# AlexanderDzhoganov/sphereflake-raytracer

Hardware: AMD Instinct MI355X
Metric: Mrays/sec into G-buffer at 1920x1080 depth-8; frame time ms (higher is better)
Workload: dtype f32

## Files before the change

### sphereflake-raytracer_amd/csrc/sf_capi.hip

```cpp
#include <hip/hip_runtime.h>

#include <cfloat>
#include <cmath>
#include <cstdlib>
#include <cstring>
#include <new>
#include <utility>
#include <vector>

#include "sf_build_id.h"
#include "sf_internal.h"
#include "sphereflake/sf.h"

extern "C" __global__ void sf_trace_wave1(FrameArgs a, uint32_t* overflow_list, uint32_t* overflow_count);
extern "C" __global__ void sf_trace_wave2(FrameArgs a, uint32_t* overflow_list, uint32_t* overflow_count);
extern "C" __global__ void sf_trace_wave4(FrameArgs a, uint32_t* overflow_list, uint32_t* overflow_count);
extern "C" __global__ void sf_trace_queue1(FrameArgs a);
extern "C" __global__ void sf_trace_queue1c(FrameArgs a);
extern "C" __global__ void sf_trace_queue1t(FrameArgs a);
extern "C" __global__ void sf_trace_frames1(FrameBatch b);
extern "C" __global__ void sf_trace_queue1g(FrameArgs a);
extern "C" __global__ void sf_trace_queue1s(FrameArgs a);
extern "C" __global__ void sf_trace_queue2(FrameArgs a);
extern "C" __global__ void sf_trace_queue4(FrameArgs a);
// ... 827 lines not shown
    a.min_t = min_t;
    a.hit_index = hidx;
    a.tile_trace = c->tile_trace;
    a.counters = c->ovf_counters;
    a.overflow_list = c->ovf_list;
    a.parity = c->parity;
    if (c->tile_trace) {
        const size_t ntr = (size_t)((c->W + 7) / 8) * ((c->H + 7) / 8);
        a.phase_sums = c->tile_trace + 3 * ntr;
    }

    uint32_t ntiles = a.tiles_x * tile_rows;
    const uint32_t blocks = (ntiles + SF_WAVES_PER_BLOCK - 1) / SF_WAVES_PER_BLOCK;
    if (p.kernel == SF_KERNEL_PER_RAY) {
        a.max_depth = 31;
        hipLaunchKernelGGL(sf_trace_ray, dim3(blocks), dim3(256), 0, s, a);
        SF_HIP(c, hipGetLastError());
    } else {
        const bool autod = p.max_depth == 0;
        bool bounded = false;
        uint32_t levels = frame_levels(c, &bounded);
        if (!autod) bounded = bounded && p.max_depth >= levels;
        a.max_depth = autod ? levels : p.max_depth;
        const size_t lds = (size_t)SF_LDS_WAVE_FLOATS(a.max_depth) * 4;
        uint32_t* cnt = c->ovf_counters + c->parity;
        const uint32_t wpb = c->waves_per_block;
        const dim3 block(64 * wpb);
        const bool front_first = (c->flags & (SF_FLAG_NO_OCCL_CULL | SF_FLAG_NO_FRONT_FIRST)) == 0u;
        const bool tie_inline = bounded && c->persistent && front_first && c->tie_inline;
        if (tie_inline) a.flags |= SF_FLAG_TIE_INLINE;
        if (c->persistent) {
            const uint32_t lean_off = SF_FLAG_DIAG_HALF | SF_FLAG_DIAG_HALF_SEL | SF_FLAG_DIAG_UNITS |
                                      SF_FLAG_DIAG_FORCE_RETRACE | SF_FLAG_PRIO_FLAT;
            const bool plain = c->lean && wpb == 1 && band_count == 1u && !a.compact && !a.packed && !a.emit_aux &&
                               !a.tile_trace;
            const bool lean_ok = plain && (a.flags & lean_off) == 0u;
            const void* kern = wpb == 1 ? (const void*)sf_trace_queue1g
                             : wpb == 2 ? (c->compact ? (const void*)sf_trace_queue2c : (const void*)sf_trace_queue2)
                                        : (const void*)sf_trace_queue4;
            const int key = (int)(wpb * 64 + a.max_depth) | (c->compact ? 1 << 20 : 0);
            if (c->occ_key != key) {
                int nb = 0;
                SF_HIP(c, hipOccupancyMaxActiveBlocksPerMultiprocessor(&nb, kern, (int)block.x, wpb * lds));
                c->occ_blocks = nb < 1 ? 1 : nb;
                c->occ_blocks_lean = c->occ_blocks;
                c->occ_blocks_pair = c->occ_blocks;
                if (wpb == 1) {
                    SF_HIP(c, hipOccupancyMaxActiveBlocksPerMultiprocessor(&nb, (const void*)sf_trace_queue1t, (int)block.x, lds));
                    c->occ_blocks_lean = nb < 1 ? 1 : nb;
                    SF_HIP(c, hipOccupancyMaxActiveBlocksPerMultiprocessor(&nb, (const void*)sf_trace_queue1, (int)block.x, lds));
                    c->occ_blocks_pair = nb < 1 ? 1 : nb;
                    SF_HIP(c, hipOccupancyMaxActiveBlocksPerMultiprocessor(&nb, (const void*)sf_trace_queue1c, (int)block.x, lds));
                    if (nb >= 1 && nb < c->occ_blocks_pair) c->occ_blocks_pair = nb;
                }
                c->occ_key = key;
            }
            const uint32_t pair_off = lean_off & ~SF_FLAG_DIAG_FORCE_RETRACE;
            const uint32_t pair_grid = (uint32_t)(c->occ_blocks_pair > c->occ_blocks_lean ? c->occ_blocks_pair
// ... 1810 lines not shown
```

### sphereflake-raytracer_amd/csrc/sf_internal.h

```cpp
#pragma once

#include <stdint.h>

#if defined(__HIPCC__) || defined(__HIP__)
#define SF_HD __host__ __device__
#else
#define SF_HD
#endif

#define SF_DEPTH_TABLE 33
#ifndef SF_OCCL_MARGIN
#define SF_OCCL_MARGIN 0x1.8p-9f
#endif
#define SF_TILE 8
#define SF_WAVES_PER_BLOCK 4
#ifndef SF_WAVES_PER_EU
#define SF_WAVES_PER_EU 8
#endif
#ifndef SF_PAIR_WAVES_PER_EU
#define SF_PAIR_WAVES_PER_EU 7
#endif
#ifndef SF_TRACE_WAVES
#define SF_TRACE_WAVES 1
#endif
#define SF_LDS_ROOT 16
#define SF_LDS_CONE 8
#define SF_LDS_PLANE 38
#define SF_LDS_COLS 27
#define SF_LDS_TABLE (SF_LDS_PLANE + 3 * SF_LDS_COLS)
#define SF_LDS_E 32
#define SF_LDS_LEVEL (SF_LDS_TABLE + SF_LDS_E + 1)
#define SF_LDS_WAVE_FLOATS(levels) (SF_LDS_ROOT + SF_LDS_CONE + ((levels) - 1) * SF_LDS_LEVEL)
#define SF_RAYS_CSTACK (3 * 64)
#define SF_LDS_RAYS_FLOATS(levels) (SF_LDS_WAVE_FLOATS((levels) + 1) + (levels) * SF_RAYS_CSTACK)

#define SF_QUEUES 32u
// ... 226 lines not shown
```

### sphereflake-raytracer_amd/csrc/sf_kernels.hip

```cpp
#include <hip/hip_runtime.h>
#include <float.h>
#include <stddef.h>
#include <stdint.h>

#include "sf_internal.h"

#pragma clang fp contract(off)

#define SF_MAX_LEVELS 31

namespace {

__device__ __forceinline__ uint64_t wave_ballot(bool p) { return __builtin_amdgcn_ballot_w64(p); }

__device__ __forceinline__ float rsqrtps_x86(float x, const uint32_t* __restrict__ lut)
{
    const uint32_t b = __float_as_uint(x);
    const uint32_t E = (b >> 23) & 0xffu;
    const uint32_t key = ((E & 1u) << 10) | ((b & 0x7fffffu) >> 13);
    const int32_t E0 = (E & 1u) ? 127 : 128;
    const int32_t k = ((int32_t)E - E0) / 2;
    uint32_t r = (uint32_t)((int32_t)lut[key] - k * (1 << 23));
    if ((b & 0x7fffffffu) > 0x7f800000u) r = b | 0x00400000u;
    else if (E == 0u) r = (b & 0x80000000u) | 0x7f800000u;
// ... 501 lines not shown
    const float tlx = sel_mask(t_lo, -__builtin_inff(), tinym);
    const float th = hb ? thx : __builtin_inff();
    const float tl = hb ? tlx : __builtin_inff();
    uint64_t exm = wave_ballot(th < T);
    const uint64_t undm = wave_ballot(sel_mask(tl, __builtin_inff(), exm) < T);
    if (undm) {
        const float te = near_root_exact(tca, d2, R2b);
        exm |= undm & wave_ballot(te < T);
    }
    return exm;
}

__device__ __forceinline__ bool child_expands(float cx, float cy, float cz, float cc, float dx, float dy, float dz,
                                              float actv, float R2b, float T, float Tfar)
{
    const float tca = (cx * dx + cy * dy) + cz * dz;
    const float d2 = cc - tca * tca;
    const float xs = R2b - d2;
    const bool hb = __builtin_fminf(__builtin_fminf(tca, xs), actv) >= 0.0f;
    const uint64_t hbm = wave_ballot(hb);
    return hbm != 0ull && lod_expands(tca, d2, xs, hb, hbm, R2b, T, Tfar) != 0ull;
}

template <bool ANYHIT, bool INDEX_ORDER = false>
__device__ __forceinline__ uint64_t accept_hits(HitState& h, uint64_t& ancm, uint32_t& status, bool flag_ties,
                                                const float4 pc, float tca, float d2, uint32_t dd, uint64_t hsm,
                                                uint32_t idx, float R2s)
{
    {
        const float xs = R2s - d2;
        float ts;
        if ((wave_ballot(!(xs >= 0x1p-96f)) & hsm) != 0ull) ts = near_root_exact(tca, d2, R2s);
        else ts = near_root_big(tca, xs);
        uint64_t accm = hsm & wave_ballot(ts < h.minT);
        if constexpr (ANYHIT) {
            uint32_t hd = (uint32_t)h.depth;
            sel_in_place(hd, dd, accm);
            h.depth = (int32_t)hd;
            return accm;
        }
        const uint64_t tie = hsm & wave_ballot(ts == h.minT);
        if constexpr (INDEX_ORDER) accm |= tie & ancm;
        else if (tie != 0ull) {
            accm |= tie & ancm;
            if (flag_ties && (tie & ~ancm) != 0ull) status |= SF_STATUS_TIE;
        }
        sel_in_place(h.minT, ts, accm);
        sel_in_place(h.cx, pc.x, accm);
        sel_in_place(h.cy, pc.y, accm);
        sel_in_place(h.cz, pc.z, accm);
        sel_in_place(h.index, idx, accm);
        uint32_t hd = (uint32_t)h.depth;
        sel_in_place(hd, dd, accm);
        h.depth = (int32_t)hd;
        ancm |= accm;
        return accm;
    }
}
template <bool ANYHIT, bool INDEX_ORDER = false>
__device__ __forceinline__ uint64_t accept_self(HitState& h, uint64_t& ancm, uint32_t& status, bool flag_ties,
                                                const float4 pc, float tca, float d2, uint32_t dd, float actv,
                                                uint32_t idx, float R2s)
{
    const uint64_t hsm = wave_ballot(__builtin_fminf(__builtin_fminf(tca, R2s - d2), actv) >= 0.0f);
    if (hsm) return accept_hits<ANYHIT, INDEX_ORDER>(h, ancm, status, flag_ties, pc, tca, d2, dd, hsm, idx, R2s);
    return 0ull;
}

template <bool ANYHIT>
__device__ __forceinline__ uint64_t occluded(float tca, float minT, float cull_t, float cull_r)
{
    float v = tca - minT;
    if constexpr (!ANYHIT) v = __builtin_fminf(v, tca - cull_t);
    return wave_ballot(v - SF_OCCL_MARGIN * tca > cull_r);
}

__device__ __forceinline__ void leaf_children(HitState& h, uint64_t& ancm, uint32_t& status, bool flag_ties,
                                              bool occl_cull, const float* tb, uint32_t Cl, float dx, float dy, float dz,
                                              float avx, uint32_t idx0, uint32_t dd, const float4 dc, const float4 dk,
                                              float cull_t)
{
    const float R2b = dc.x, R2s = dc.y, T = dc.w, Tfar = dk.z, cull_r = dk.y;
    while (Cl) {
        const uint32_t p = __builtin_ctz(Cl);
        __asm__("s_bitset0_b32 %0, %1" : "+s"(Cl) : "s"(p));
        const uint32_t c = p & 15u;
        lds_fence();
        const float4 pc = *reinterpret_cast<const float4*>(tb + c * 4u);
        const float tca = (pc.x * dx + pc.y * dy) + pc.z * dz;
        const float d2 = pc.w - tca * tca;
        const bool hs = __builtin_fminf(__builtin_fminf(tca, R2s - d2), avx) >= 0.0f;
        const uint64_t hsm = wave_ballot(hs);
        if (hsm == 0ull) continue;
        uint64_t amx = lod_expands(tca, d2, R2b - d2, hs, hsm, R2b, T, Tfar);
        if (amx == 0ull) continue;
        if (occl_cull) {
            amx &= ~occluded<false>(tca, h.minT, cull_t, cull_r);
            if (amx == 0ull) continue;
        }
        ancm &= ~accept_hits<false>(h, ancm, status, flag_ties, pc, tca, d2, dd, amx, idx0 + c, R2s);
    }
}

template <class Ray>
__device__ __forceinline__ void leaf_children_pair(Ray& ra, Ray& rb, uint64_t& ancA, uint64_t& ancB, uint32_t& status,
                                                   bool flag_ties, bool occl_cull, const float* tb, uint32_t Cl,
                                                   float avxA, float avxB, uint32_t idx0, uint32_t dd, const float4 dc,
                                                   const float4 dk, float cull_t)
{
    const float R2b = dc.x, R2s = dc.y, T = dc.w, Tfar = dk.z, cull_r = dk.y;
    while (Cl) {
        const uint32_t p = __builtin_ctz(Cl);
        __asm__("s_bitset0_b32 %0, %1" : "+s"(Cl) : "s"(p));
        const uint32_t c = p & 15u;
        lds_fence();
        const float4 pc = *reinterpret_cast<const float4*>(tb + c * 4u);
        const float tcaA = (pc.x * ra.dx + pc.y * ra.dy) + pc.z * ra.dz;
        const float tcaB = (pc.x * rb.dx + pc.y * rb.dy) + pc.z * rb.dz;
        const float d2A = pc.w - tcaA * tcaA;
        const float d2B = pc.w - tcaB * tcaB;
        const bool hsA = __builtin_fminf(__builtin_fminf(tcaA, R2s - d2A), avxA) >= 0.0f;
        const bool hsB = __builtin_fminf(__builtin_fminf(tcaB, R2s - d2B), avxB) >= 0.0f;
        const uint64_t hsmA = wave_ballot(hsA), hsmB = wave_ballot(hsB);
        if ((hsmA | hsmB) == 0ull) continue;
        uint64_t amxA = hsmA ? lod_expands(tcaA, d2A, R2b - d2A, hsA, hsmA, R2b, T, Tfar) : 0ull;
        uint64_t amxB = hsmB ? lod_expands(tcaB, d2B, R2b - d2B, hsB, hsmB, R2b, T, Tfar) : 0ull;
        if ((amxA | amxB) == 0ull) continue;
        if (occl_cull) {
            amxA &= ~occluded<false>(tcaA, ra.h.minT, cull_t, cull_r);
            amxB &= ~occluded<false>(tcaB, rb.h.minT, cull_t, cull_r);
        }
        if (amxA) ancA &= ~accept_hits<false>(ra.h, ancA, status, flag_ties, pc, tcaA, d2A, dd, amxA, idx0 + c, R2s);
        if (amxB) ancB &= ~accept_hits<false>(rb.h, ancB, status, flag_ties, pc, tcaB, d2B, dd, amxB, idx0 + c, R2s);
    }
}

struct LeafLevel {
    float4 dc;
    bool on;
};
struct ChildBuild {
    float x, y, z, w;
    uint32_t M, front;
    float4 dtc;
    bool leaf_level;
};
template <bool KP_CONE = false>
__device__ __forceinline__ ChildBuild build_children(const DeviceConsts* K, const TraverseLds& L, const BuildLane& B,
                                                     const float4 pc, const float* col, uint32_t cs, uint32_t ko,
                                                     float kp, uint32_t index_order)
{
    lds_fence();
    const float3 p0 = *reinterpret_cast<const float3*>(col);
    const float3 p1 = *reinterpret_cast<const float3*>(col + cs);
    const float3 p2 = *reinterpret_cast<const float3*>(col + 2u * cs);
    const float4 cn = *reinterpret_cast<const float4*>(L.cone());
// ... 244 lines not shown
    __device__ __forceinline__ int32_t depth(uint32_t flags) const
    {
        int32_t seed = -1;
        if ((flags & (SF_FLAG_NO_OCCL_CULL | SF_FLAG_NO_DEPTH_SEED)) == 0u) {
            const int32_t w = __builtin_amdgcn_readfirstlane(word);
            const int32_t o = __builtin_amdgcn_readfirstlane(own);
            const int32_t m = o > w ? o : w;
            seed = (m > 0 ? m : 0) & 31;
        }
        return __builtin_amdgcn_readfirstlane(seed);
    }
};
__device__ __forceinline__ int32_t stats_word(const FrameArgs& a)
{
    return __hip_atomic_load(&a.stats[0], __ATOMIC_RELAXED, __HIP_MEMORY_SCOPE_AGENT);
}

__device__ __forceinline__ uint32_t split_mask(uint32_t q, uint32_t idxB)
{
    const uint32_t m9 = (0x111u << ((q - idxB) & 3u)) & 0x1ffu;
    return m9 | (m9 << 16);
}

template <bool COMPACT = false, bool SPLIT = false, bool SHADOW = false, bool LEAFNODES = !(COMPACT || SPLIT || SHADOW)>
__device__ __forceinline__ void traverse_ray(const DeviceConsts* __restrict__ K, const float* root, float* __restrict__ Lbase,
                                             const float4 bcol, uint32_t levels, float dx, float dy, float dz, bool valid,
                                             HitState& h, int32_t& maxd, uint32_t& status, uint32_t K_flags,
                                             uint64_t* phase_sums = nullptr, uint32_t axl = 36u,
                                             uint64_t* tile_counts = nullptr, uint32_t split_q = 0u,
                                             uint32_t split_depth = 0u, int32_t seed = -1, float bound = FLT_MAX)
{
    const uint32_t lane = threadIdx.x & 63u;
    const TraverseLds L{ Lbase };
    const bool cone_cull = (K_flags & SF_FLAG_NO_CONE_CULL) == 0u;
    const bool occl_cull = (K_flags & SF_FLAG_NO_OCCL_CULL) == 0u;
    const bool front_first = (K_flags & (SF_FLAG_NO_OCCL_CULL | SF_FLAG_NO_FRONT_FIRST)) == 0u;
    SF_STAMP_DECL;

    reset_hit(h, SHADOW ? bound : FLT_MAX);
    uint64_t ancm = 0ull;

    const float rcx = root[9], rcy = root[10], rcz = root[11];
    const float rcc = (rcx * rcx + rcy * rcy) + rcz * rcz;
    uint64_t ex0m;
    {
        const float4 dt0 = depth_consts(K, 0u);
        const float tca = (rcx * dx + rcy * dy) + rcz * dz;
        const float d2 = rcc - tca * tca;
        const bool hb = valid && tca >= 0.0f && d2 <= dt0.x;
        const uint64_t hbm = wave_ballot(hb);
        if (hbm == 0ull) return;
        ex0m = lod_expands(tca, d2, dt0.x - d2, hb, hbm, dt0.x, dt0.w, depth_word_at(K, 0u, 6u));
        if (ex0m == 0ull) return;
    }
    maxd = 0;

    {
        const float ax = readlane_f(dx, axl), ay = readlane_f(dy, axl), az = readlane_f(dz, axl);
        stage_cone(L, lane, cone_cull, ax, ay, az, [&] { return cone_s2m(dx, dy, dz, ax, ay, az); });
    }

    float cull_t = depth_consts(K, (uint32_t)(seed > 0 ? seed : 0) + 1u).w;

    const BuildLane B = build_lane(bcol, lane, build_child(lane));

    uint32_t d = 0;
    uint32_t idxB = 1;

    auto self_test = [&](const float4 pc, float tca, float d2, uint32_t dd, float actv, uint32_t idx,
                         float R2s) -> uint64_t {
        return accept_self<SHADOW>(h, ancm, status, front_first, pc, tca, d2, dd, actv, idx, R2s);
    };

    const uint32_t lv32 = __builtin_amdgcn_readfirstlane(levels << 5);
    const uint32_t index_order = front_first ? 0u : 0x1ffu;
    auto expand = [&](const float4 pc, const float* col, uint32_t cs, uint32_t d, float actv,
                      float* tb, uint32_t ko, float kp, LeafLevel& lf) -> uint32_t {
        d = __builtin_amdgcn_readfirstlane(d);
        SF_COUNT(0, 1);
        SF_COUNT(7, __builtin_popcountll(wave_ballot(actv >= 0.0f)));
        const ChildBuild cb = build_children(K, L, B, pc, col, cs, ko, kp, index_order);
        lf.dc = cb.dtc;
        lf.on = false;
        if (ko < lv32) {
            *reinterpret_cast<float3*>(tb + B.slot) = make_float3(cb.x, cb.y, cb.z);
            *(B.bc == 3u ? tb + B.slot + 3u : L.cone() + 5u) = cb.w;
            lf.on = cb.leaf_level;
            return (cb.M & cb.front) | ((cb.M & ~cb.front) << 16);
        }
        {
            const float R2b = cb.dtc.x, T = cb.dtc.w, Tfar = depth_word_at(K, ko, 6u);
            uint32_t M = cb.M;
            while (M) {
                const uint32_t i = __builtin_ctz(M);
// ... 83 lines not shown
            if (occl_cull) {
                amx = exm & ~occluded<SHADOW>(tca, h.minT, cull_t, cull_r);
                SF_COUNT(13, 1);
                SF_COUNT(12, amx == 0ull ? 1 : 0);
                if (amx == 0ull) continue;
            }
            float avx = sel_mask(-1.0f, __builtin_inff(), amx);
            const uint64_t acc = self_test(pc, tca, d2, d + 1u, avx, idxB + c, dc.y);
            SF_STAMP(4);
            if constexpr (SHADOW) {
                if (acc != 0ull) {
                    amx &= ~acc;
                    avx = sel_mask(avx, -1.0f, acc);
                    actv = sel_mask(actv, -1.0f, acc);
                    sel_in_place(actbits, 0u, acc);
                    if (wave_ballot(actbits != 0u) == 0ull) break;
                    if (amx == 0ull) continue;
                }
            }
            if (wave_ballot(pc.w > dk.x) != 0ull) {
                SF_COUNT(4, 1);
                SF_COUNT(8, 1);
                SF_COUNT(9, __builtin_popcountll(amx));
                ancm &= wave_ballot(h.depth != (int32_t)d + 1);
                continue;
            }
            const float* const col = tcur + SF_LDS_PLANE + 3u * c;
            auto push = [&]() {
                stk_pc = writelane_s(C, d, stk_pc);
                stk_ix = writelane_s(idxB, d, stk_ix);
                {
                    const uint32_t bit = 2u << d;
                    uint32_t ab = actbits & ~bit;
                    sel_in_place(ab, ab | bit, amx);
                    actbits = ab;
                }
                idxB = 9u * (idxB + c) + 1u;
                d += 1u;
                actv = avx;
                tcur += SF_LDS_LEVEL;
                kofs += 1u << 5;
            };
            LeafLevel lf;
            if constexpr (LEAFNODES) {
                SF_STAMP(1);
                const uint32_t Cn = expand(pc, col, SF_LDS_COLS, d + 1u, avx, tcur + SF_LDS_LEVEL, kofs + (1u << 5),
                                           readlane_f(tca, axl), lf);
                if (lf.on && (Cn == 0u || (int32_t)d + 2 <= (maxd > seed ? maxd : seed))) {
                    SF_COUNT(10, 1);
                    SF_COUNT(11, __builtin_popcount(Cn));
                    leaf_children(h, ancm, status, front_first, occl_cull, tcur + SF_LDS_LEVEL, Cn, dx, dy, dz, avx,
                                  9u * (idxB + c) + 1u, d + 2u, lf.dc, depth_consts_at(K, kofs + (1u << 5) + 16u), cull_t);
                    ancm &= wave_ballot(h.depth != (int32_t)d + 1);
                    SF_STAMP(6);
                    continue;
                }
                push();
                C = Cn;
            } else {
                push();
                SF_STAMP(1);
                C = expand(pc, col, SF_LDS_COLS, d, avx, tcur, kofs, readlane_f(tca, axl), lf);
            }
            if constexpr (SPLIT) {
                if (d + 1u == split_depth) C &= split_mask(split_q, idxB);
            }
            if constexpr (LEAFNODES) R2c = lf.dc.x;
            else R2c = depth_consts_at(K, kofs).x;
            if (COMPACT && C != 0u) {
                __builtin_amdgcn_sched_barrier(0);
                const uint64_t actm = wave_ballot(avx > 0.0f);
                const uint32_t na = (uint32_t)__builtin_popcountll(actm);
                const uint32_t M = (C | (C >> 16)) & 0x1ffu;
                if (na <= 7u && __builtin_popcount(M) >= 3) {
                    const float R2b = depth_consts(K, d + 1u).x;
                    const uint32_t rank = __builtin_amdgcn_mbcnt_hi((uint32_t)(actm >> 32),
// ... 4 lines not shown
                    uint32_t ln = lane;
                    __asm__ volatile("" : "+v"(ln));
                    const uint32_t g = (ln * 37u) >> 8;
                    const uint32_t sl = ln - 7u * g;
                    const float4 q = *reinterpret_cast<const float4*>(sc + 4u * sl);
                    const bool ok = sl < na && g < 9u && ((M >> g) & 1u) != 0u;
                    const uint32_t gi = g < 9u ? g : 8u;
                    const float4 cg = *reinterpret_cast<const float4*>(L.table(d) + gi * 4u);
                    const float tca = (cg.x * q.x + cg.y * q.y) + cg.z * q.z;
                    const float d2 = cg.w - tca * tca;
                    const float xs = R2b - d2;
                    const uint64_t bal =
                        wave_ballot(__builtin_fminf(__builtin_fminf(tca, xs), ok ? __builtin_inff() : -1.0f) >= 0.0f);
                    const uint32_t kk = ln < 9u ? ln : 0u;
                    const uint64_t grp = (bal >> (7u * kk)) & 0x7full;
                    const uint32_t hitm = (uint32_t)wave_ballot(ln < 9u && grp != 0ull) & 0x1ffu;
                    const uint32_t keep = __builtin_amdgcn_readfirstlane(hitm);
                    C &= keep | (keep << 16);
                }
            }
            SF_STAMP(6);
            continue;
        }
        ancm &= wave_ballot(h.depth != (int32_t)d);
        if (d == 0u) break;
        d -= 1u;
        tcur -= SF_LDS_LEVEL;
        kofs -= 1u << 5;
        R2c = depth_consts_at(K, kofs).x;
        {
            const uint32_t pw = __builtin_amdgcn_readlane(stk_pc, d);
            C = pw;
            idxB = (uint32_t)__builtin_amdgcn_readlane(stk_ix, d);
        }
        actv = ((actbits >> d) & 1u) ? __builtin_inff() : -1.0f;
        SF_STAMP(5);
    }
    h.hit = h.depth >= 0;
    SF_STAMP_FLUSH(phase_sums);
#ifdef SF_COUNTS
    if (tile_counts) {
        auto sat = [](uint64_t v) { return v > 0xffffull ? 0xffffull : v; };
        *tile_counts = sat(ph_sum[0]) | (sat(ph_sum[1]) << 16) | (sat(ph_sum[1] - ph_sum[2]) << 32) | (sat(ph_sum[8]) << 48);
    }
#else
    (void)tile_counts;
#endif
}

struct PairRay {
    float dx, dy, dz;
    HitState h;
    float actv;
    uint32_t actbits;
};

__device__ __forceinline__ void traverse_pair(const DeviceConsts* __restrict__ K, const float* root, float* __restrict__ Lbase,
                                              const float4 bcol, uint32_t levels, PairRay& ra, PairRay& rb, bool validA,
                                              bool validB, int32_t& maxd, uint32_t& status, uint32_t K_flags,
                                              int32_t seed)
{
    const uint32_t lane = threadIdx.x & 63u;
    const uint32_t axl = 39u;
    const TraverseLds L{ Lbase };
    const bool cone_cull = (K_flags & SF_FLAG_NO_CONE_CULL) == 0u;
    const bool occl_cull = (K_flags & SF_FLAG_NO_OCCL_CULL) == 0u;
    const bool front_first = (K_flags & (SF_FLAG_NO_OCCL_CULL | SF_FLAG_NO_FRONT_FIRST)) == 0u;

    reset_hit(ra.h, FLT_MAX);
    reset_hit(rb.h, FLT_MAX);
    uint64_t ancA = 0ull, ancB = 0ull;

    const float rcx = root[9], rcy = root[10], rcz = root[11];
    const float rcc = (rcx * rcx + rcy * rcy) + rcz * rcz;
    uint64_t ex0A = 0ull, ex0B = 0ull;
    {
        const float4 dt0 = depth_consts(K, 0u);
        const float Tfar0 = depth_word_at(K, 0u, 6u);
        auto root_lod = [&](const PairRay& r, bool valid) -> uint64_t {
            const float tca = (rcx * r.dx + rcy * r.dy) + rcz * r.dz;
            const float d2 = rcc - tca * tca;
            const bool hb = valid && tca >= 0.0f && d2 <= dt0.x;
            const uint64_t hbm = wave_ballot(hb);
            if (hbm == 0ull) return 0ull;
            return lod_expands(tca, d2, dt0.x - d2, hb, hbm, dt0.x, dt0.w, Tfar0);
        };
        ex0A = root_lod(ra, validA);
        ex0B = root_lod(rb, validB);
        if ((ex0A | ex0B) == 0ull) return;
    }
    maxd = 0;

    const float ax = readlane_f(ra.dx, axl), ay = readlane_f(ra.dy, axl), az = readlane_f(ra.dz, axl);
    {
        auto s2m_of = [&](const PairRay& r) -> float {
            const float cx_ = r.dy * az - r.dz * ay, cy_ = r.dz * ax - r.dx * az, cz_ = r.dx * ay - r.dy * ax;
            const float s2 = (cx_ * cx_ + cy_ * cy_) + cz_ * cz_;
            const bool fwd = (r.dx * ax + r.dy * ay) + r.dz * az > 0.0f;
            return fwd ? s2 : 1.0f;
        };
        uint32_t ln = lane;
        __asm__ volatile("" : "+v"(ln));
        stage_cone(L, ln, cone_cull, ax, ay, az, [&] { return __builtin_fmaxf(s2m_of(ra), s2m_of(rb)); });
    }

    float cull_t = depth_consts(K, (uint32_t)(seed > 0 ? seed : 0) + 1u).w;

    const BuildLane B = build_lane(bcol, lane, build_child(lane));

    uint32_t d = 0;
    uint32_t idxB = 1;

    auto self_test = [&](PairRay& r, uint64_t& ancm, const float4 pc, float tca, float d2, uint32_t dd, float actv,
                         uint32_t idx, float R2s) {
        accept_self<false>(r.h, ancm, status, front_first, pc, tca, d2, dd, actv, idx, R2s);
    };

    const uint32_t lv32 = __builtin_amdgcn_readfirstlane(levels << 5);
    const uint32_t index_order = front_first ? 0u : 0x1ffu;
    auto expand = [&](const float4 pc, const float* col, uint32_t cs, float* tb, uint32_t ko, float kp, auto kp_cone,
                      float actvA, float actvB, LeafLevel& lf) -> uint32_t {
        const ChildBuild cb = build_children<decltype(kp_cone)::value>(K, L, B, pc, col, cs, ko, kp, index_order);
        lf.dc = cb.dtc;
        lf.on = false;
        if (ko < lv32) {
            *reinterpret_cast<float3*>(tb + B.slot) = make_float3(cb.x, cb.y, cb.z);
            *(B.bc == 3u ? tb + B.slot + 3u : L.cone() + 5u) = cb.w;
            lf.on = cb.leaf_level;
            return (cb.M & cb.front) | ((cb.M & ~cb.front) << 16);
        }
        {
            const float R2b = cb.dtc.x, T = cb.dtc.w, Tfar = depth_word_at(K, ko, 6u);
            uint32_t M = cb.M;
            while (M) {
                const uint32_t i = __builtin_ctz(M);
                M &= ~(1u << i);
                const float cx = readlane_f(cb.x, 32u + i), cy = readlane_f(cb.y, 32u + i);
                const float cz = readlane_f(cb.z, 32u + i), cc = readlane_f(cb.w, 32u + i);
                auto passes = [&](const PairRay& r, float actv) -> bool {
                    return child_expands(cx, cy, cz, cc, r.dx, r.dy, r.dz, actv, R2b, T, Tfar);
                };
                if (passes(ra, actvA) || passes(rb, actvB)) {
                    status |= SF_STATUS_OVERFLOW;
                    break;
                }
            }
            return 0u;
        }
    };

    uint32_t stk_pc = 0u, stk_ix = 0u;
    float* tcur = L.table(0u);
    uint32_t kofs = 1u << 5;
    float R2c = depth_consts_at(K, kofs).x;
    uint32_t C = 0u;

    auto dfs_one = [&](const uint32_t base) {
        for (;;) {
            d = __builtin_amdgcn_readfirstlane(d);
            if (C) {
                const uint32_t p = __builtin_ctz(C);
                __asm__("s_bitset0_b32 %0, %1" : "+s"(C) : "s"(p));
                const uint32_t c = p & 15u;
                const float4 dc = depth_consts_at(K, kofs);
                lds_fence();
                const float4 pc = *reinterpret_cast<const float4*>(tcur + c * 4u);
                const float tca = (pc.x * ra.dx + pc.y * ra.dy) + pc.z * ra.dz;
                const float d2 = pc.w - tca * tca;
                const float xs = R2c - d2;
                const bool hb = __builtin_fminf(__builtin_fminf(tca, xs), ra.actv) >= 0.0f;
                const uint64_t hbm = wave_ballot(hb);
                if (hbm == 0ull) continue;
                const float4 dk = depth_consts_at(K, kofs + 16u);
                const float Tfar = dk.z;
                const float cull_r = dk.y;
                const uint64_t exm = lod_expands(tca, d2, xs, hb, hbm, dc.x, dc.w, Tfar);
                if (exm == 0ull) continue;
                if ((int32_t)d + 1 > maxd) {
                    maxd = (int32_t)d + 1;
                    if ((int32_t)d + 1 > seed) cull_t = depth_consts_at(K, kofs + (1u << 5)).w;
                }
                uint64_t amx = exm;
                if (occl_cull) {
                    amx = exm & ~occluded<false>(tca, ra.h.minT, cull_t, cull_r);
                    if (amx == 0ull) continue;
                }
                const float avx = sel_mask(-1.0f, __builtin_inff(), amx);
                self_test(ra, ancA, pc, tca, d2, d + 1u, avx, idxB + c, dc.y);
                if (wave_ballot(pc.w > dk.x) != 0ull) {
                    ancA &= wave_ballot(ra.h.depth != (int32_t)d + 1);
                    continue;
                }
                LeafLevel lf;
                const uint32_t Cn = expand(pc, tcur + SF_LDS_PLANE + 3u * c, SF_LDS_COLS, tcur + SF_LDS_LEVEL,
                                           kofs + (1u << 5), 0.0f, BoolC<true>(), avx, rb.actv, lf);
                if (lf.on && (Cn == 0u || (int32_t)d + 2 <= (maxd > seed ? maxd : seed))) {
                    leaf_children(ra.h, ancA, status, front_first, occl_cull, tcur + SF_LDS_LEVEL, Cn, ra.dx, ra.dy, ra.dz,
                                  avx, 9u * (idxB + c) + 1u, d + 2u, lf.dc, depth_consts_at(K, kofs + (1u << 5) + 16u), cull_t);
                    ancA &= wave_ballot(ra.h.depth != (int32_t)d + 1);
                    continue;
                }
                stk_pc = writelane_s(C, d, stk_pc);
                stk_ix = writelane_s(idxB, d, stk_ix);
                {
                    const uint32_t bit = 2u << d;
                    uint32_t ab = ra.actbits & ~bit;
                    sel_in_place(ab, ab | bit, amx);
                    ra.actbits = ab;
                }
                idxB = 9u * (idxB + c) + 1u;
                d += 1u;
                ra.actv = avx;
                tcur += SF_LDS_LEVEL;
                kofs += 1u << 5;
                C = Cn;
                R2c = lf.dc.x;
                continue;
            }
            ancA &= wave_ballot(ra.h.depth != (int32_t)d);
            if (d == base) break;
            d -= 1u;
            tcur -= SF_LDS_LEVEL;
            kofs -= 1u << 5;
            R2c = depth_consts_at(K, kofs).x;
            C = (uint32_t)__builtin_amdgcn_readlane(stk_pc, d);
            idxB = (uint32_t)__builtin_amdgcn_readlane(stk_ix, d);
            ra.actv = ((ra.actbits >> d) & 1u) ? __builtin_inff() : -1.0f;
        }
    };
    auto exchange = [&](const uint64_t mB) {
        {
            __asm__("s_mov_b64 vcc, exec\n\t"
                    "s_mov_b64 exec, %22\n\t"
                    "v_swap_b32 %0, %11\n\t"
                    "v_swap_b32 %1, %12\n\t"
                    "v_swap_b32 %2, %13\n\t"
                    "v_swap_b32 %3, %14\n\t"
                    "v_swap_b32 %4, %15\n\t"
                    "v_swap_b32 %5, %16\n\t"
                    "v_swap_b32 %6, %17\n\t"
                    "v_swap_b32 %7, %18\n\t"
                    "v_swap_b32 %8, %19\n\t"
                    "v_swap_b32 %9, %20\n\t"
                    "v_swap_b32 %10, %21\n\t"
                    "s_mov_b64 exec, vcc"
                    : "+v"(ra.dx), "+v"(ra.dy), "+v"(ra.dz), "+v"(ra.h.minT), "+v"(ra.h.cx), "+v"(ra.h.cy), "+v"(ra.h.cz),
                      "+v"(ra.h.index), "+v"(ra.h.depth), "+v"(ra.actv), "+v"(ra.actbits), "+v"(rb.dx), "+v"(rb.dy),
                      "+v"(rb.dz), "+v"(rb.h.minT), "+v"(rb.h.cx), "+v"(rb.h.cy), "+v"(rb.h.cz), "+v"(rb.h.index),
                      "+v"(rb.h.depth), "+v"(rb.actv), "+v"(rb.actbits)
                    : "s"(mB)
                    : "vcc");
            const uint64_t x = (ancA ^ ancB) & mB;
            ancA ^= x;
            ancB ^= x;
        }
    };
    auto one_ray_subtree = [&](const uint64_t mB) {
        if (mB) exchange(mB);
        dfs_one(d);
        if (mB) exchange(mB);
    };
    auto one_ray_leaves = [&](const uint64_t mB, const float* tb, uint32_t Cl, float avx, uint32_t idx0, uint32_t dd,
                              const LeafLevel& lf) {
        if (mB) exchange(mB);
        leaf_children(ra.h, ancA, status, front_first, occl_cull, tb, Cl, ra.dx, ra.dy, ra.dz, avx, idx0, dd, lf.dc, depth_consts_at(K, kofs + (1u << 5) + 16u),
                      cull_t);
        if (mB) exchange(mB);
    };

    {
        lds_fence();
        const float4 pc = *reinterpret_cast<const float4*>(L.root());
        const float R2s0 = depth_consts(K, 0u).y;
        auto enter_root = [&](PairRay& r, uint64_t& ancm, uint64_t ex0m) -> float {
            r.actv = sel_mask(-1.0f, __builtin_inff(), ex0m);
            r.actbits = 0u;
            sel_in_place(r.actbits, 1u, ex0m);
            const float tca = (pc.x * r.dx + pc.y * r.dy) + pc.z * r.dz;
            const float d2 = pc.w - tca * tca;
            self_test(r, ancm, pc, tca, d2, 0u, r.actv, 0u, R2s0);
            return tca;
        };
        const float tcaA = enter_root(ra, ancA, ex0A);
        enter_root(rb, ancB, ex0B);
        LeafLevel lf0;
        if (!__builtin_amdgcn_readfirstlane((int)(pc.w > depth_leaf(K, 0u))))
            C = expand(pc, L.root() + 4u, 4u, tcur, kofs, readlane_f(tcaA, axl), BoolC<false>(), ra.actv, rb.actv, lf0);
    }
    if ((ex0A & ex0B) == 0ull) {
        one_ray_subtree(ex0B);
        C = 0u;
    }

    for (;;) {
        d = __builtin_amdgcn_readfirstlane(d);
        if (C) {
            const uint32_t p = __builtin_ctz(C);
            __asm__("s_bitset0_b32 %0, %1" : "+s"(C) : "s"(p));
            const uint32_t c = p & 15u;
            const float4 dc = depth_consts_at(K, kofs);
            lds_fence();
            const float4 pc = *reinterpret_cast<const float4*>(tcur + c * 4u);
            const float tcaA = (pc.x * ra.dx + pc.y * ra.dy) + pc.z * ra.dz;
            const float tcaB = (pc.x * rb.dx + pc.y * rb.dy) + pc.z * rb.dz;
            const float d2A = pc.w - tcaA * tcaA;
            const float d2B = pc.w - tcaB * tcaB;
            const float xsA = R2c - d2A;
// ... 2 lines not shown
            const bool hbB = __builtin_fminf(__builtin_fminf(tcaB, xsB), rb.actv) >= 0.0f;
            const uint64_t hbmA = wave_ballot(hbA), hbmB = wave_ballot(hbB);
            if ((hbmA | hbmB) == 0ull) continue;
            const float4 dk = depth_consts_at(K, kofs + 16u);
            const float Tfar = dk.z;
            const float cull_r = dk.y;
            const uint64_t exmA = hbmA ? lod_expands(tcaA, d2A, xsA, hbA, hbmA, dc.x, dc.w, Tfar) : 0ull;
            const uint64_t exmB = hbmB ? lod_expands(tcaB, d2B, xsB, hbB, hbmB, dc.x, dc.w, Tfar) : 0ull;
            if ((exmA | exmB) == 0ull) continue;
            if ((int32_t)d + 1 > maxd) {
                maxd = (int32_t)d + 1;
                if ((int32_t)d + 1 > seed) cull_t = depth_consts_at(K, kofs + (1u << 5)).w;
            }
            uint64_t amxA = exmA, amxB = exmB;
            if (occl_cull) {
                const float vA = __builtin_fminf(tcaA - ra.h.minT, tcaA - cull_t);
                const float vB = __builtin_fminf(tcaB - rb.h.minT, tcaB - cull_t);
                amxA = exmA & ~wave_ballot(vA - SF_OCCL_MARGIN * tcaA > cull_r);
                amxB = exmB & ~wave_ballot(vB - SF_OCCL_MARGIN * tcaB > cull_r);
                if ((amxA | amxB) == 0ull) continue;
            }
            const float avxA = sel_mask(-1.0f, __builtin_inff(), amxA);
            const float avxB = sel_mask(-1.0f, __builtin_inff(), amxB);
            self_test(ra, ancA, pc, tcaA, d2A, d + 1u, avxA, idxB + c, dc.y);
            self_test(rb, ancB, pc, tcaB, d2B, d + 1u, avxB, idxB + c, dc.y);
            if (wave_ballot(pc.w > dk.x) != 0ull) {
                ancA &= wave_ballot(ra.h.depth != (int32_t)d + 1);
                ancB &= wave_ballot(rb.h.depth != (int32_t)d + 1);
                continue;
            }
            LeafLevel lf;
            const uint32_t Cn = expand(pc, tcur + SF_LDS_PLANE + 3u * c, SF_LDS_COLS, tcur + SF_LDS_LEVEL, kofs + (1u << 5),
                                       readlane_f(tcaA, axl), BoolC<false>(), avxA, avxB, lf);
            if (lf.on && (Cn == 0u || (int32_t)d + 2 <= (maxd > seed ? maxd : seed))) {
                if ((amxA & amxB) == 0ull)
                    one_ray_leaves(amxB, tcur + SF_LDS_LEVEL, Cn, sel_mask(avxA, __builtin_inff(), amxB),
                                   9u * (idxB + c) + 1u, d + 2u, lf);
                else
                    leaf_children_pair(ra, rb, ancA, ancB, status, front_first, occl_cull, tcur + SF_LDS_LEVEL, Cn, avxA,
                                       avxB, 9u * (idxB + c) + 1u, d + 2u, lf.dc, depth_consts_at(K, kofs + (1u << 5) + 16u), cull_t);
                ancA &= wave_ballot(ra.h.depth != (int32_t)d + 1);
                ancB &= wave_ballot(rb.h.depth != (int32_t)d + 1);
                continue;
            }
            stk_pc = writelane_s(C, d, stk_pc);
            stk_ix = writelane_s(idxB, d, stk_ix);
            {
                const uint32_t bit = 2u << d;
                uint32_t abA = ra.actbits & ~bit, abB = rb.actbits & ~bit;
                sel_in_place(abA, abA | bit, amxA);
                sel_in_place(abB, abB | bit, amxB);
                ra.actbits = abA;
                rb.actbits = abB;
            }
            idxB = 9u * (idxB + c) + 1u;
            d += 1u;
            ra.actv = avxA;
            rb.actv = avxB;
            tcur += SF_LDS_LEVEL;
            kofs += 1u << 5;
            C = Cn;
            R2c = lf.dc.x;
            if ((amxA & amxB) == 0ull) one_ray_subtree(amxB);
            continue;
        }
        ancA &= wave_ballot(ra.h.depth != (int32_t)d);
        ancB &= wave_ballot(rb.h.depth != (int32_t)d);
        if (d == 0u) break;
        d -= 1u;
        tcur -= SF_LDS_LEVEL;
        kofs -= 1u << 5;
        R2c = depth_consts_at(K, kofs).x;
        C = (uint32_t)__builtin_amdgcn_readlane(stk_pc, d);
        idxB = (uint32_t)__builtin_amdgcn_readlane(stk_ix, d);
        ra.actv = ((ra.actbits >> d) & 1u) ? __builtin_inff() : -1.0f;
        rb.actv = ((rb.actbits >> d) & 1u) ? __builtin_inff() : -1.0f;
    }
    ra.h.hit = ra.h.depth >= 0;
    rb.h.hit = rb.h.depth >= 0;
}

struct Tile {
    uint32_t x, y, orow;
    bool valid;
};

template <bool LEAN = false>
__device__ __forceinline__ Tile tile_of(const FrameArgs& a, uint32_t tile, uint32_t lane, uint32_t part = 0u, uint32_t txm_lean = 0u)
{
    auto divmod = [](uint32_t n, uint32_t D, uint32_t m, uint32_t& r) {
        uint32_t q = __umulhi(n, m);
        r = n - q * D;
        if (r >= D) {
            q += 1u;
            r -= D;
        }
        return q;
// ... 195 lines not shown
    at = a;
#endif
}

template <bool FIXUP, class Prefetch = NoPrefetch, bool COMPACT = false, bool SPLIT = false, bool LEAN = false>
__device__ __forceinline__ TileStats trace_tile(const FrameArgs& a, float* __restrict__ L, const float4 bcol, uint32_t tile,
                                                uint32_t levels, uint32_t* overflow_list, uint32_t* overflow_count,
                                                uint32_t part = 0u, const Prefetch& pre = Prefetch(), uint32_t fl = ~0u,
                                                uint32_t slot = 0u, const DepthSeed seen = DepthSeed())
{
    const uint32_t flags = fl == ~0u ? a.flags : fl;
    const DeviceConsts* __restrict__ K = a.consts;
    const uint32_t lane = threadIdx.x & 63u;
    if constexpr (LEAN) {
        static_assert(!FIXUP && !SPLIT && !COMPACT, "the lean tile is the plain persistent loop's");
        const FrameConsts fc = frame_consts(K);
        const Tile t = tile_of<true>(a, tile, lane, 0u, fc.tx_magic);
        float dx, dy, dz;
        ray_dir(a, (float)t.x, (float)t.y, dx, dy, dz, K->lut, &fc, &t.valid);
        const int32_t seed = seen.depth(flags);
        HitState h;
        int32_t maxd = -1;
        uint32_t status = 0u;
        traverse_ray<>(K, a.root, L, bcol, levels, dx, dy, dz, t.valid, h, maxd, status, flags, nullptr, 36u, nullptr, 0u, 0u,
                       seed);
        const bool overflowed = status != 0u;
        const bool retrace = __builtin_amdgcn_readfirstlane((int)(status == SF_STATUS_TIE && (flags & SF_FLAG_TIE_INLINE))) != 0;
        pre(retrace);
        FrameArgs ae;
        kernarg_frame(ae, a);
        if (overflowed && !retrace) {
            const uint32_t slot = wave_fetch_add(ae.counters + ae.parity, 1u);
            ae.overflow_list[slot] = tile;
        }
        write_pixel<true>(ae, t, dx, dy, dz, h, K->lut);
        TileStats st;
        st.maxd = maxd;
        st.seed = seed;
        st.closest = t.valid ? h.minT : FLT_MAX;
        st.overflowed = overflowed;
        return st;
    }
    if (flags & SF_FLAG_DIAG_HALF) part = (flags & SF_FLAG_DIAG_HALF_SEL) ? 2u : 1u;
    const bool sub = SPLIT && !FIXUP && (flags & SF_FLAG_SUBTREE) != 0u && part >= SF_PART_QUARTER0;
    const Tile t = tile_of(a, tile, lane, sub ? 0u : part);
    const uint64_t t_start = a.tile_trace ? __builtin_amdgcn_s_memrealtime() : 0ull;
    const uint64_t c_start = (!FIXUP && a.tile_cost) ? __builtin_amdgcn_s_memtime() : 0ull;
    float dx, dy, dz;
// ... 2572 lines not shown
```

Baseline: 46040.

## Derive tie ancestry from heap index and skip empty stack levels on pop

```diff
diff --git a/sphereflake-raytracer_amd/csrc/sf_capi.hip b/sphereflake-raytracer_amd/csrc/sf_capi.hip
--- a/sphereflake-raytracer_amd/csrc/sf_capi.hip
+++ b/sphereflake-raytracer_amd/csrc/sf_capi.hip
@@ -873,9 +873,16 @@
         uint32_t levels = frame_levels(c, &bounded);
         if (!autod) bounded = bounded && p.max_depth >= levels;
         a.max_depth = autod ? levels : p.max_depth;
-        const size_t lds = (size_t)SF_LDS_WAVE_FLOATS(a.max_depth) * 4;
+        const uint32_t wpb = c->waves_per_block;
+        const bool plain_ask = c->persistent && c->lean && wpb == 1 && band_count == 1u && !a.compact && !a.packed &&
+                               !a.emit_aux && !a.tile_trace;
+        if (plain_ask && autod && !c->levels_override && a.max_depth > SF_HEAPTIE_LEVELS &&
+            *(volatile int32_t*)c->h_depth < 0) {
+            a.max_depth = SF_HEAPTIE_LEVELS;
+            bounded = false;
+        }
+        const size_t lds =(size_t)SF_LDS_WAVE_FLOATS(a.max_depth) * 4;
         uint32_t* cnt = c->ovf_counters + c->parity;
-        const uint32_t wpb = c->waves_per_block;
         const dim3 block(64 * wpb);
         const bool front_first = (c->flags & (SF_FLAG_NO_OCCL_CULL | SF_FLAG_NO_FRONT_FIRST)) == 0u;
         const bool tie_inline = bounded && c->persistent && front_first && c->tie_inline;
@@ -883,8 +890,7 @@
         if (c->persistent) {
             const uint32_t lean_off = SF_FLAG_DIAG_HALF | SF_FLAG_DIAG_HALF_SEL | SF_FLAG_DIAG_UNITS |
                                       SF_FLAG_DIAG_FORCE_RETRACE | SF_FLAG_PRIO_FLAT;
-            const bool plain = c->lean && wpb == 1 && band_count == 1u && !a.compact && !a.packed && !a.emit_aux &&
-                               !a.tile_trace;
+            const bool plain = plain_ask && a.max_depth <= SF_HEAPTIE_LEVELS;
             const bool lean_ok = plain && (a.flags & lean_off) == 0u;
             const void* kern = wpb == 1 ? (const void*)sf_trace_queue1g
                              : wpb == 2 ? (c->compact ? (const void*)sf_trace_queue2c : (const void*)sf_trace_queue2)
diff --git a/sphereflake-raytracer_amd/csrc/sf_internal.h b/sphereflake-raytracer_amd/csrc/sf_internal.h
--- a/sphereflake-raytracer_amd/csrc/sf_internal.h
+++ b/sphereflake-raytracer_amd/csrc/sf_internal.h
@@ -12,6 +12,7 @@
 #ifndef SF_OCCL_MARGIN
 #define SF_OCCL_MARGIN 0x1.8p-9f
 #endif
+#define SF_HEAPTIE_LEVELS 11u
 #define SF_TILE 8
 #define SF_WAVES_PER_BLOCK 4
 #ifndef SF_WAVES_PER_EU
diff --git a/sphereflake-raytracer_amd/csrc/sf_kernels.hip b/sphereflake-raytracer_amd/csrc/sf_kernels.hip
--- a/sphereflake-raytracer_amd/csrc/sf_kernels.hip
+++ b/sphereflake-raytracer_amd/csrc/sf_kernels.hip
@@ -547,7 +547,19 @@
     return hbm != 0ull && lod_expands(tca, d2, xs, hb, hbm, R2b, T, Tfar) != 0ull;
 }
 
-template <bool ANYHIT, bool INDEX_ORDER = false>
+__device__ __forceinline__ uint64_t heap_ancestor_lanes(uint32_t hindex, int32_t hdepth, uint32_t idx)
+{
+    uint64_t m = 0ull;
+    uint32_t n = __builtin_amdgcn_readfirstlane(idx);
+    for (;;) {
+        m |= wave_ballot(hindex == n);
+        if (n == 0u) break;
+        n = (n - 1u) / 9u;
+    }
+    return m & wave_ballot(hdepth >= 0);
+}
+
+template <bool ANYHIT, bool INDEX_ORDER = false, bool HEAPTIE = false>
 __device__ __forceinline__ uint64_t accept_hits(HitState& h, uint64_t& ancm, uint32_t& status, bool flag_ties,
                                                 const float4 pc, float tca, float d2, uint32_t dd, uint64_t hsm,
                                                 uint32_t idx, float R2s)
@@ -567,8 +579,10 @@
         const uint64_t tie = hsm & wave_ballot(ts == h.minT);
         if constexpr (INDEX_ORDER) accm |= tie & ancm;
         else if (tie != 0ull) {
-            accm |= tie & ancm;
-            if (flag_ties && (tie & ~ancm) != 0ull) status |= SF_STATUS_TIE;
+            uint64_t anc = ancm;
+            if constexpr (HEAPTIE) anc = heap_ancestor_lanes(h.index, h.depth, idx);
+            accm |= tie & anc;
+            if (flag_ties && (tie & ~anc) != 0ull) status |= SF_STATUS_TIE;
         }
         sel_in_place(h.minT, ts, accm);
         sel_in_place(h.cx, pc.x, accm);
@@ -578,17 +592,17 @@
         uint32_t hd = (uint32_t)h.depth;
         sel_in_place(hd, dd, accm);
         h.depth = (int32_t)hd;
-        ancm |= accm;
+        if constexpr (!HEAPTIE) ancm |= accm;
         return accm;
     }
 }
-template <bool ANYHIT, bool INDEX_ORDER = false>
+template <bool ANYHIT, bool INDEX_ORDER = false, bool HEAPTIE = false>
 __device__ __forceinline__ uint64_t accept_self(HitState& h, uint64_t& ancm, uint32_t& status, bool flag_ties,
                                                 const float4 pc, float tca, float d2, uint32_t dd, float actv,
                                                 uint32_t idx, float R2s)
 {
     const uint64_t hsm = wave_ballot(__builtin_fminf(__builtin_fminf(tca, R2s - d2), actv) >= 0.0f);
-    if (hsm) return accept_hits<ANYHIT, INDEX_ORDER>(h, ancm, status, flag_ties, pc, tca, d2, dd, hsm, idx, R2s);
+    if (hsm) return accept_hits<ANYHIT, INDEX_ORDER, HEAPTIE>(h, ancm, status, flag_ties, pc, tca, d2, dd, hsm, idx, R2s);
     return 0ull;
 }
 
@@ -600,6 +614,7 @@
     return wave_ballot(v - SF_OCCL_MARGIN * tca > cull_r);
 }
 
+template <bool HEAPTIE = false>
 __device__ __forceinline__ void leaf_children(HitState& h, uint64_t& ancm, uint32_t& status, bool flag_ties,
                                               bool occl_cull, const float* tb, uint32_t Cl, float dx, float dy, float dz,
                                               float avx, uint32_t idx0, uint32_t dd, const float4 dc, const float4 dk,
@@ -623,12 +638,13 @@
             amx &= ~occluded<false>(tca, h.minT, cull_t, cull_r);
             if (amx == 0ull) continue;
         }
-        ancm &= ~accept_hits<false>(h, ancm, status, flag_ties, pc, tca, d2, dd, amx, idx0 + c, R2s);
+        const uint64_t accm = accept_hits<false, false, HEAPTIE>(h, ancm, status, flag_ties, pc, tca, d2, dd, amx, idx0 + c, R2s);
+        if constexpr (!HEAPTIE) ancm &= ~accm;
     }
 }
 
 template <class Ray>
-__device__ __forceinline__ void leaf_children_pair(Ray& ra, Ray& rb, uint64_t& ancA, uint64_t& ancB, uint32_t& status,
+__device__ __forceinline__ void leaf_children_pair(Ray& ra, Ray& rb, uint32_t& status,
                                                    bool flag_ties, bool occl_cull, const float* tb, uint32_t Cl,
                                                    float avxA, float avxB, uint32_t idx0, uint32_t dd, const float4 dc,
                                                    const float4 dk, float cull_t)
@@ -655,8 +671,9 @@
             amxA &= ~occluded<false>(tcaA, ra.h.minT, cull_t, cull_r);
             amxB &= ~occluded<false>(tcaB, rb.h.minT, cull_t, cull_r);
         }
-        if (amxA) ancA &= ~accept_hits<false>(ra.h, ancA, status, flag_ties, pc, tcaA, d2A, dd, amxA, idx0 + c, R2s);
-        if (amxB) ancB &= ~accept_hits<false>(rb.h, ancB, status, flag_ties, pc, tcaB, d2B, dd, amxB, idx0 + c, R2s);
+        uint64_t none = 0ull;
+        if (amxA) accept_hits<false, false, true>(ra.h, none, status, flag_ties, pc, tcaA, d2A, dd, amxA, idx0 + c, R2s);
+        if (amxB) accept_hits<false, false, true>(rb.h, none, status, flag_ties, pc, tcaB, d2B, dd, amxB, idx0 + c, R2s);
     }
 }
 
@@ -947,7 +964,8 @@
     return m9 | (m9 << 16);
 }
 
-template <bool COMPACT = false, bool SPLIT = false, bool SHADOW = false, bool LEAFNODES = !(COMPACT || SPLIT || SHADOW)>
+template <bool COMPACT = false, bool SPLIT = false, bool SHADOW = false, bool LEAFNODES = !(COMPACT || SPLIT || SHADOW),
+          bool HEAPTIE = false>
 __device__ __forceinline__ void traverse_ray(const DeviceConsts* __restrict__ K, const float* root, float* __restrict__ Lbase,
                                              const float4 bcol, uint32_t levels, float dx, float dy, float dz, bool valid,
                                              HitState& h, int32_t& maxd, uint32_t& status, uint32_t K_flags,
@@ -963,6 +981,7 @@
     SF_STAMP_DECL;
 
     reset_hit(h, SHADOW ? bound : FLT_MAX);
+    static_assert(!HEAPTIE || (LEAFNODES && !COMPACT), "the heap-index tie rule is the lean tile loop's");
     uint64_t ancm = 0ull;
 
     const float rcx = root[9], rcy = root[10], rcz = root[11];
@@ -994,7 +1013,7 @@
 
     auto self_test = [&](const float4 pc, float tca, float d2, uint32_t dd, float actv, uint32_t idx,
                          float R2s) -> uint64_t {
-        return accept_self<SHADOW>(h, ancm, status, front_first, pc, tca, d2, dd, actv, idx, R2s);
+        return accept_self<SHADOW, false, HEAPTIE>(h, ancm, status, front_first, pc, tca, d2, dd, actv, idx, R2s);
     };
 
     const uint32_t lv32 = __builtin_amdgcn_readfirstlane(levels << 5);
@@ -1124,7 +1143,7 @@
                 SF_COUNT(4, 1);
                 SF_COUNT(8, 1);
                 SF_COUNT(9, __builtin_popcountll(amx));
-                ancm &= wave_ballot(h.depth != (int32_t)d + 1);
+                if constexpr (!HEAPTIE) ancm &= wave_ballot(h.depth != (int32_t)d + 1);
                 continue;
             }
             const float* const col = tcur + SF_LDS_PLANE + 3u * c;
@@ -1151,9 +1170,9 @@
                 if (lf.on && (Cn == 0u || (int32_t)d + 2 <= (maxd > seed ? maxd : seed))) {
                     SF_COUNT(10, 1);
                     SF_COUNT(11, __builtin_popcount(Cn));
-                    leaf_children(h, ancm, status, front_first, occl_cull, tcur + SF_LDS_LEVEL, Cn, dx, dy, dz, avx,
+                    leaf_children<HEAPTIE>(h, ancm, status, front_first, occl_cull, tcur + SF_LDS_LEVEL, Cn, dx, dy, dz, avx,
                                   9u * (idxB + c) + 1u, d + 2u, lf.dc, depth_consts_at(K, kofs + (1u << 5) + 16u), cull_t);
-                    ancm &= wave_ballot(h.depth != (int32_t)d + 1);
+                    if constexpr (!HEAPTIE) ancm &= wave_ballot(h.depth != (int32_t)d + 1);
                     SF_STAMP(6);
                     continue;
                 }
@@ -1204,11 +1223,19 @@
             SF_STAMP(6);
             continue;
         }
-        ancm &= wave_ballot(h.depth != (int32_t)d);
-        if (d == 0u) break;
-        d -= 1u;
-        tcur -= SF_LDS_LEVEL;
-        kofs -= 1u << 5;
+        if constexpr (HEAPTIE) {
+            const uint32_t nz = (uint32_t)wave_ballot(stk_pc != 0u) & ((1u << d) - 1u);
+            if (nz == 0u) break;
+            d = 31u - (uint32_t)__builtin_clz(nz);
+            tcur = L.table(0u) + d * SF_LDS_LEVEL;
+            kofs = (d + 1u) << 5;
+        } else {
+            ancm &= wave_ballot(h.depth != (int32_t)d);
+            if (d == 0u) break;
+            d -= 1u;
+            tcur -= SF_LDS_LEVEL;
+            kofs -= 1u << 5;
+        }
         R2c = depth_consts_at(K, kofs).x;
         {
             const uint32_t pw = __builtin_amdgcn_readlane(stk_pc, d);
@@ -1251,7 +1278,6 @@
 
     reset_hit(ra.h, FLT_MAX);
     reset_hit(rb.h, FLT_MAX);
-    uint64_t ancA = 0ull, ancB = 0ull;
 
     const float rcx = root[9], rcy = root[10], rcz = root[11];
     const float rcc = (rcx * rcx + rcy * rcy) + rcz * rcz;
@@ -1293,9 +1319,16 @@
     uint32_t d = 0;
     uint32_t idxB = 1;
 
-    auto self_test = [&](PairRay& r, uint64_t& ancm, const float4 pc, float tca, float d2, uint32_t dd, float actv,
-                         uint32_t idx, float R2s) {
-        accept_self<false>(r.h, ancm, status, front_first, pc, tca, d2, dd, actv, idx, R2s);
+    auto self_test = [&](PairRay& r, const float4 pc, float tca, float d2, uint32_t dd, float actv, uint32_t idx,
+                         float R2s) {
+        uint64_t none = 0ull;
+        accept_self<false, false, true>(r.h, none, status, front_first, pc, tca, d2, dd, actv, idx, R2s);
+    };
+    auto leaves_one = [&](const float* tb, uint32_t Cl, float avx, uint32_t idx0, uint32_t dd, const float4 dc,
+                          const float4 dk) {
+        uint64_t none = 0ull;
+        leaf_children<true>(ra.h, none, status, front_first, occl_cull, tb, Cl, ra.dx, ra.dy, ra.dz, avx, idx0, dd, dc, dk,
+                            cull_t);
     };
 
     const uint32_t lv32 = __builtin_amdgcn_readfirstlane(levels << 5);
@@ -1336,6 +1369,18 @@
     uint32_t kofs = 1u << 5;
     float R2c = depth_consts_at(K, kofs).x;
     uint32_t C = 0u;
+
+    auto pop_to = [&](const uint32_t base) -> bool {
+        const uint32_t nz = (uint32_t)wave_ballot(stk_pc != 0u) & ((1u << d) - (1u << base));
+        d = nz ? 31u - (uint32_t)__builtin_clz(nz) : base;
+        tcur = L.table(0u) + d * SF_LDS_LEVEL;
+        kofs = (d + 1u) << 5;
+        if (nz == 0u) return false;
+        R2c = depth_consts_at(K, kofs).x;
+        C = (uint32_t)__builtin_amdgcn_readlane(stk_pc, d);
+        idxB = (uint32_t)__builtin_amdgcn_readlane(stk_ix, d);
+        return true;
+    };
 
     auto dfs_one = [&](const uint32_t base) {
         for (;;) {
@@ -1368,18 +1413,14 @@
                     if (amx == 0ull) continue;
                 }
                 const float avx = sel_mask(-1.0f, __builtin_inff(), amx);
-                self_test(ra, ancA, pc, tca, d2, d + 1u, avx, idxB + c, dc.y);
-                if (wave_ballot(pc.w > dk.x) != 0ull) {
-                    ancA &= wave_ballot(ra.h.depth != (int32_t)d + 1);
-                    continue;
-                }
+                self_test(ra, pc, tca, d2, d + 1u, avx, idxB + c, dc.y);
+                if (wave_ballot(pc.w > dk.x) != 0ull) continue;
                 LeafLevel lf;
                 const uint32_t Cn = expand(pc, tcur + SF_LDS_PLANE + 3u * c, SF_LDS_COLS, tcur + SF_LDS_LEVEL,
                                            kofs + (1u << 5), 0.0f, BoolC<true>(), avx, rb.actv, lf);
                 if (lf.on && (Cn == 0u || (int32_t)d + 2 <= (maxd > seed ? maxd : seed))) {
-                    leaf_children(ra.h, ancA, status, front_first, occl_cull, tcur + SF_LDS_LEVEL, Cn, ra.dx, ra.dy, ra.dz,
-                                  avx, 9u * (idxB + c) + 1u, d + 2u, lf.dc, depth_consts_at(K, kofs + (1u << 5) + 16u), cull_t);
-                    ancA &= wave_ballot(ra.h.depth != (int32_t)d + 1);
+                    leaves_one(tcur + SF_LDS_LEVEL, Cn, avx, 9u * (idxB + c) + 1u, d + 2u, lf.dc,
+                               depth_consts_at(K, kofs + (1u << 5) + 16u));
                     continue;
                 }
                 stk_pc = writelane_s(C, d, stk_pc);
@@ -1399,14 +1440,7 @@
                 R2c = lf.dc.x;
                 continue;
             }
-            ancA &= wave_ballot(ra.h.depth != (int32_t)d);
-            if (d == base) break;
-            d -= 1u;
-            tcur -= SF_LDS_LEVEL;
-            kofs -= 1u << 5;
-            R2c = depth_consts_at(K, kofs).x;
-            C = (uint32_t)__builtin_amdgcn_readlane(stk_pc, d);
-            idxB = (uint32_t)__builtin_amdgcn_readlane(stk_ix, d);
+            if (!pop_to(base)) break;
             ra.actv = ((ra.actbits >> d) & 1u) ? __builtin_inff() : -1.0f;
         }
     };
@@ -1432,9 +1466,6 @@
                       "+v"(rb.h.depth), "+v"(rb.actv), "+v"(rb.actbits)
                     : "s"(mB)
                     : "vcc");
-            const uint64_t x = (ancA ^ ancB) & mB;
-            ancA ^= x;
-            ancB ^= x;
         }
     };
     auto one_ray_subtree = [&](const uint64_t mB) {
@@ -1445,8 +1476,7 @@
     auto one_ray_leaves = [&](const uint64_t mB, const float* tb, uint32_t Cl, float avx, uint32_t idx0, uint32_t dd,
                               const LeafLevel& lf) {
         if (mB) exchange(mB);
-        leaf_children(ra.h, ancA, status, front_first, occl_cull, tb, Cl, ra.dx, ra.dy, ra.dz, avx, idx0, dd, lf.dc, depth_consts_at(K, kofs + (1u << 5) + 16u),
-                      cull_t);
+        leaves_one(tb, Cl, avx, idx0, dd, lf.dc, depth_consts_at(K, kofs + (1u << 5) + 16u));
         if (mB) exchange(mB);
     };
 
@@ -1454,17 +1484,17 @@
         lds_fence();
         const float4 pc = *reinterpret_cast<const float4*>(L.root());
         const float R2s0 = depth_consts(K, 0u).y;
-        auto enter_root = [&](PairRay& r, uint64_t& ancm, uint64_t ex0m) -> float {
+        auto enter_root = [&](PairRay& r, uint64_t ex0m) -> float {
             r.actv = sel_mask(-1.0f, __builtin_inff(), ex0m);
             r.actbits = 0u;
             sel_in_place(r.actbits, 1u, ex0m);
             const float tca = (pc.x * r.dx + pc.y * r.dy) + pc.z * r.dz;
             const float d2 = pc.w - tca * tca;
-            self_test(r, ancm, pc, tca, d2, 0u, r.actv, 0u, R2s0);
+            self_test(r, pc, tca, d2, 0u, r.actv, 0u, R2s0);
             return tca;
         };
-        const float tcaA = enter_root(ra, ancA, ex0A);
-        enter_root(rb, ancB, ex0B);
+        const float tcaA = enter_root(ra, ex0A);
+        enter_root(rb, ex0B);
         LeafLevel lf0;
         if (!__builtin_amdgcn_readfirstlane((int)(pc.w > depth_leaf(K, 0u))))
             C = expand(pc, L.root() + 4u, 4u, tcur, kofs, readlane_f(tcaA, axl), BoolC<false>(), ra.actv, rb.actv, lf0);
@@ -1513,13 +1543,9 @@
             }
             const float avxA = sel_mask(-1.0f, __builtin_inff(), amxA);
             const float avxB = sel_mask(-1.0f, __builtin_inff(), amxB);
-            self_test(ra, ancA, pc, tcaA, d2A, d + 1u, avxA, idxB + c, dc.y);
-            self_test(rb, ancB, pc, tcaB, d2B, d + 1u, avxB, idxB + c, dc.y);
-            if (wave_ballot(pc.w > dk.x) != 0ull) {
-                ancA &= wave_ballot(ra.h.depth != (int32_t)d + 1);
-                ancB &= wave_ballot(rb.h.depth != (int32_t)d + 1);
-                continue;
-            }
+            self_test(ra, pc, tcaA, d2A, d + 1u, avxA, idxB + c, dc.y);
+            self_test(rb, pc, tcaB, d2B, d + 1u, avxB, idxB + c, dc.y);
+            if (wave_ballot(pc.w > dk.x) != 0ull) continue;
             LeafLevel lf;
             const uint32_t Cn = expand(pc, tcur + SF_LDS_PLANE + 3u * c, SF_LDS_COLS, tcur + SF_LDS_LEVEL, kofs + (1u << 5),
                                        readlane_f(tcaA, axl), BoolC<false>(), avxA, avxB, lf);
@@ -1528,10 +1554,8 @@
                     one_ray_leaves(amxB, tcur + SF_LDS_LEVEL, Cn, sel_mask(avxA, __builtin_inff(), amxB),
                                    9u * (idxB + c) + 1u, d + 2u, lf);
                 else
-                    leaf_children_pair(ra, rb, ancA, ancB, status, front_first, occl_cull, tcur + SF_LDS_LEVEL, Cn, avxA,
+                    leaf_children_pair(ra, rb, status, front_first, occl_cull, tcur + SF_LDS_LEVEL, Cn, avxA,
                                        avxB, 9u * (idxB + c) + 1u, d + 2u, lf.dc, depth_consts_at(K, kofs + (1u << 5) + 16u), cull_t);
-                ancA &= wave_ballot(ra.h.depth != (int32_t)d + 1);
-                ancB &= wave_ballot(rb.h.depth != (int32_t)d + 1);
                 continue;
             }
             stk_pc = writelane_s(C, d, stk_pc);
@@ -1555,15 +1579,7 @@
             if ((amxA & amxB) == 0ull) one_ray_subtree(amxB);
             continue;
         }
-        ancA &= wave_ballot(ra.h.depth != (int32_t)d);
-        ancB &= wave_ballot(rb.h.depth != (int32_t)d);
-        if (d == 0u) break;
-        d -= 1u;
-        tcur -= SF_LDS_LEVEL;
-        kofs -= 1u << 5;
-        R2c = depth_consts_at(K, kofs).x;
-        C = (uint32_t)__builtin_amdgcn_readlane(stk_pc, d);
-        idxB = (uint32_t)__builtin_amdgcn_readlane(stk_ix, d);
+        if (!pop_to(0u)) break;
         ra.actv = ((ra.actbits >> d) & 1u) ? __builtin_inff() : -1.0f;
         rb.actv = ((rb.actbits >> d) & 1u) ? __builtin_inff() : -1.0f;
     }
@@ -1805,8 +1821,8 @@
         HitState h;
         int32_t maxd = -1;
         uint32_t status = 0u;
-        traverse_ray<>(K, a.root, L, bcol, levels, dx, dy, dz, t.valid, h, maxd, status, flags, nullptr, 36u, nullptr, 0u, 0u,
-                       seed);
+        traverse_ray<false, false, false, true, true>(K, a.root, L, bcol, levels, dx, dy, dz, t.valid, h, maxd, status, flags,
+                                                      nullptr, 36u, nullptr, 0u, 0u, seed);
         const bool overflowed = status != 0u;
         const bool retrace = __builtin_amdgcn_readfirstlane((int)(status == SF_STATUS_TIE && (flags & SF_FLAG_TIE_INLINE))) != 0;
         pre(retrace);
```

New measurement: 46640, median of 6. +1.3%, better.
